# lachlants/denet

Hardware: AMD Instinct MI355X
Metric: images/sec train step, DeNet-34 skip 512x512 (higher is better)
Workload: dtype f32

## Files before the change

### denet_amd/csrc/winograd.hip

```cpp
#include "wino.h"
#include "bn_pointwise.h"
#include "../../include/denet_hip.h"

namespace {

template <int MO>
__global__ __launch_bounds__(256) void wino_input_kernel(const float* __restrict__ x, float* __restrict__ V, int N, int H,
                                                         int W, int C, int TH, int TW, long T, int up) {
    using WT = Wino<MO>;
    constexpr int TS = WT::TS;
    const int c4n = C / 4;
    const long idx = (long)blockIdx.x * 256 + threadIdx.x;
    if (idx >= T * c4n) return;
    const int c4 = (int)(idx % c4n);
    const long t = idx / c4n;
    const int tx = (int)(t % TW);
    const int ty = (int)((t / TW) % TH);
    const int n = (int)(t / ((long)TW * TH));
    const f32x4 z = {0.f, 0.f, 0.f, 0.f};
    f32x4 tt[TS][TS];
#pragma unroll
    for (int j = 0; j < TS; ++j) {
        const int ix = MO * tx - 1 + j;
        f32x4 d[TS];
#pragma unroll
        for (int i = 0; i < TS; ++i) {
            const int iy = MO * ty - 1 + i;
            const bool ok = ((unsigned)iy < (unsigned)H) && ((unsigned)ix < (unsigned)W);
            d[i] = ok ? ld4(x + (((long)n * (H >> up) + (iy >> up)) * (W >> up) + (ix >> up)) * C + c4 * 4) : z;
        }
        wino_input_col<MO>(d, tt, j);
    }
    wino_input_store<MO>(tt, V, T, t, C, c4 * 4);
}

struct BnFoldDev {
    const float* x;
    const float* aux;
    const float* y;
    const float* gamma;
    const float* beta;
    const float* mean;
    const float* invstd;
    const float* coef;
    float* out;
    int relu;
};

template <int MO, bool BWD>
struct PrepLds {
    static constexpr int BT = 4;
    static constexpr int CQ = 8;
    static constexpr int PB = BT * MO;
    static constexpr int PP = PB + 2;
    static constexpr int NT = BT * BT * CQ;
    static constexpr int PS = CQ + 1;
    static constexpr size_t LDS = (size_t)PP * PP * PS * sizeof(f32x4);
};

template <int MO, bool BWD>
__global__ __launch_bounds__(128) void wino_prep_lds_kernel(BnFoldDev f, float* __restrict__ V, float* __restrict__ dM, int N,
                                                            int H, int W, int C, int TH, int TW, long T, int BH, int BW) {
    using WT = Wino<MO>;
    using PL = PrepLds<MO, BWD>;
    static_assert(PL::NT == 128, "launch bounds");
    constexpr int TS = WT::TS, BT = PL::BT, CQ = PL::CQ, PB = PL::PB, PP = PL::PP, NT = PL::NT, PS = PL::PS;
    extern __shared__ __attribute__((aligned(16))) unsigned char prep_smem[];
    f32x4* patch = (f32x4*)prep_smem;
    const int tid = threadIdx.x;
    const int cq = tid % CQ;
    const int cblk = blockIdx.y;
    const int c = (cblk * CQ + cq) * 4;
    int b = blockIdx.x;
    const int bx = b % BW; b /= BW;
    const int by = b % BH;
    const int n = b / BH;
    const f32x4 z = {0.f, 0.f, 0.f, 0.f};
    BnQuad bq;
    bn_quad_load<false, true>(bq, f.gamma, f.beta, f.mean, f.invstd, c);
    if (BWD) bn_quad_load_coef(bq, f.coef, C, c);
    const int y0 = by * PB - 1, x0 = bx * PB - 1;
    constexpr int SLOTS = NT / CQ;
    constexpr int ROUNDS = (PP * PP + SLOTS - 1) / SLOTS;
    constexpr int UB = 7;
    for (int r0 = 0; r0 < ROUNDS; r0 += UB) {
        f32x4 xv[UB], av[UB], yv[UB];
        long off[UB];
        int pix[UB];
        bool ok[UB], inner[UB];
#pragma unroll
        for (int u = 0; u < UB; ++u) {
            const int p = (r0 + u) * SLOTS + tid / CQ;
            const int py = p / PP, px = p - py * PP;
            const int iy = y0 + py, ix = x0 + px;
            pix[u] = p;
            ok[u] = p < PP * PP && ((unsigned)iy < (unsigned)H) && ((unsigned)ix < (unsigned)W);
            inner[u] = py >= 1 && py <= PB && px >= 1 && px <= PB;
            off[u] = ok[u] ? (((long)n * H + iy) * W + ix) * C + c : (long)c;
            xv[u] = ld4(f.x + off[u]);
            if (BWD || f.aux) av[u] = ld4(f.aux + off[u]);
            if (BWD && f.relu && f.y) yv[u] = ld4(f.y + off[u]);
        }
#pragma unroll
        for (int u = 0; u < UB; ++u) {
            f32x4 d;
            if (!BWD) {
                d = bn_forward(bq, xv[u], f.aux != nullptr, av[u], f.relu);
                if (ok[u] && inner[u]) *(f32x4*)(f.out + off[u]) = d;
            } else {
                f32x4 g = av[u];
                if (f.relu) g = f.y ? bn_mask_y(g, yv[u]) : bn_mask_x(bq, g, xv[u]);
                d = bn_backward(bq, g, xv[u]);
                if (ok[u] && inner[u] && f.out) *(f32x4*)(f.out + off[u]) = g;
            }
            if (pix[u] < PP * PP) patch[pix[u] * PS + cq] = ok[u] ? d : z;
        }
    }
    __syncthreads();
    const int tl = tid / CQ;
    const int tyl = tl / BT, txl = tl - tyl * BT;
    const int ty = by * BT + tyl, tx = bx * BT + txl;
    if (ty >= TH || tx >= TW) return;
    const long t = ((long)n * TH + ty) * TW + tx;
    {
        f32x4 tt[TS][TS];
#pragma unroll
        for (int j = 0; j < TS; ++j) {
            f32x4 d[TS];
#pragma unroll
            for (int i = 0; i < TS; ++i) d[i] = patch[((MO * tyl + i) * PP + MO * txl + j) * PS + cq];
            wino_input_col<MO>(d, tt, j);
        }
        wino_input_store<MO>(tt, V, T, t, C, c);
    }
    if (BWD) {
        f32x4 a[TS][MO];
#pragma unroll
        for (int j = 0; j < MO; ++j) {
            f32x4 d[MO];
#pragma unroll
            for (int i = 0; i < MO; ++i) d[i] = patch[((MO * tyl + 1 + i) * PP + MO * txl + 1 + j) * PS + cq];
            wino_dout_col<MO>(d, a, j);
        }
        wino_dout_store<MO>(a, dM, T, t, C, c);
    }
}

template <int MO, bool BWD>
int launch_prep_lds(const BnFoldDev& f, float* V, float* dM, int N, int H, int W, int C, int TH, int TW, long T, hipStream_t stream) {
    using PL = PrepLds<MO, BWD>;
    static bool attr_set[DENET_MAX_DEVICES] = {};
    const hipError_t e = denet_allow_dynamic_lds((const void*)wino_prep_lds_kernel<MO, BWD>, (int)PL::LDS, attr_set);
    if (e != hipSuccess) {
        denet_set_error("conv_wino fold: hipFuncSetAttribute(%zu B LDS): %s", PL::LDS, hipGetErrorString(e));
        return -(int)e;
    }
    const int BH = (TH + PL::BT - 1) / PL::BT, BW = (TW + PL::BT - 1) / PL::BT;
    hipLaunchKernelGGL((wino_prep_lds_kernel<MO, BWD>), dim3((unsigned)(N * BH * BW), (unsigned)(C / (4 * PL::CQ))), dim3(PL::NT),
                       PL::LDS, stream, f, V, dM, N, H, W, C, TH, TW, T, BH, BW);
    return DENET_OK;
}

template <int MO>
__global__ __launch_bounds__(256) void wino_filter_kernel(const float* __restrict__ w, float* __restrict__ U, int K, int C) {
    using WT = Wino<MO>;
    constexpr int TS = WT::TS;
    const long idx = (long)blockIdx.x * 256 + threadIdx.x;
    if (idx >= (long)K * C) return;
    const int c = (int)(idx % C);
    const int k = (int)(idx / C);
    float g[3][3];
#pragma unroll
    for (int r = 0; r < 3; ++r)
#pragma unroll
        for (int s = 0; s < 3; ++s) g[r][s] = w[(((long)k * 3 + r) * 3 + s) * C + c];
    float u[TS][TS];
    wino_filter_transform<MO>(g, u);
    const long KC = (long)K * C;
#pragma unroll
    for (int i = 0; i < TS; ++i)
#pragma unroll
        for (int j = 0; j < TS; ++j) U[(long)(TS * i + j) * KC + (long)k * C + c] = u[i][j];
}

template <int MO>
__global__ __launch_bounds__(256) void wino_filter_dgrad_kernel(const float* __restrict__ w, float* __restrict__ U, int K,
                                                                int C) {
    using WT = Wino<MO>;
    constexpr int TS = WT::TS;
    __shared__ float tile[TS * TS][16][17];
    const int kl = threadIdx.x >> 4, cl = threadIdx.x & 15;
    const int k0 = blockIdx.y * 16, c0 = blockIdx.x * 16;
    {
        const int k = k0 + kl, c = c0 + cl;
        float g[3][3];
#pragma unroll
        for (int r = 0; r < 3; ++r)
#pragma unroll
            for (int q = 0; q < 3; ++q) g[r][q] = w[(((long)k * 3 + (2 - r)) * 3 + (2 - q)) * C + c];
        float u[TS][TS];
        wino_filter_transform<MO>(g, u);
#pragma unroll
        for (int i = 0; i < TS; ++i)
#pragma unroll
            for (int j = 0; j < TS; ++j) tile[TS * i + j][cl][kl] = u[i][j];
    }
    __syncthreads();
    const long KC = (long)K * C;
    const int co = threadIdx.x >> 4, ko = threadIdx.x & 15;
#pragma unroll
    for (int xi = 0; xi < TS * TS; ++xi) U[(long)xi * KC + (long)(c0 + co) * K + k0 + ko] = tile[xi][co][ko];
}

template <int MO>
__global__ __launch_bounds__(256) void wino_output_kernel(const float* __restrict__ Mx, const float* __restrict__ bias,
                                                          const float* __restrict__ add, float* __restrict__ y, int N,
                                                          int H, int W, int K, int TH, int TW, long T, int relu,
                                                          double* __restrict__ stats, BnFoldDev bs) {
    using WT = Wino<MO>;
    constexpr int TS = WT::TS;
    __shared__ double red[2][256][4];
    const int k4n = K / 4;
    const long idx = (long)blockIdx.x * 256 + threadIdx.x;
    const bool valid = idx < T * k4n;
    const f32x4 z = {0.f, 0.f, 0.f, 0.f};
    double dsum[4] = {0.0, 0.0, 0.0, 0.0}, dsq[4] = {0.0, 0.0, 0.0, 0.0};
    if (valid) {
        const int k4 = (int)(idx % k4n);
        const long t = idx / k4n;
        const int tx = (int)(t % TW);
        const int ty = (int)((t / TW) % TH);
        const int n = (int)(t / ((long)TW * TH));
        f32x4 s[MO][TS];
#pragma unroll
        for (int j = 0; j < TS; ++j) {
            f32x4 m[TS];
#pragma unroll
            for (int i = 0; i < TS; ++i) m[i] = ld4(Mx + ((long)(TS * i + j) * T + t) * K + k4 * 4);
            wino_output_col<MO>(m, s, j);
        }
        f32x4 b = z;
        if (bias) b = ld4(bias + k4 * 4);
        BnQuad bq = {};
        if (bs.x) bn_quad_load<true, true>(bq, bs.gamma, bs.beta, bs.mean, bs.invstd, k4 * 4);
#pragma unroll
        for (int i = 0; i < MO; ++i) {
            f32x4 ssum = z, ssq = z;
#pragma unroll
            for (int j = 0; j < MO; ++j) {
                f32x4 acc = wino_output_at<MO>(s[i], j);
                if (MO * ty + i >= H || MO * tx + j >= W) continue;
                const long o = (((long)n * H + MO * ty + i) * W + MO * tx + j) * K + k4 * 4;
                acc += b;
                if (add) acc += ld4(add + o);
                if (relu) {
                    acc[0] = fmaxf(acc[0], 0.f);
                    acc[1] = fmaxf(acc[1], 0.f);
                    acc[2] = fmaxf(acc[2], 0.f);
                    acc[3] = fmaxf(acc[3], 0.f);
                }
                *(f32x4*)(y + o) = acc;
                if (bs.x) {
                    const f32x4 xv = ld4(bs.x + o);
                    f32x4 g = acc;
                    if (bs.relu) g = bs.y ? bn_mask_y(g, ld4(bs.y + o)) : bn_mask_x(bq, g, xv);
                    ssum += g;
                    ssq += g * bn_xhat(bq, xv);
                } else {
                    ssum += acc;
                    ssq += acc * acc;
                }
            }
            if (stats) {
#pragma unroll
                for (int c = 0; c < 4; ++c) {
                    dsum[c] += (double)ssum[c];
                    dsq[c] += (double)ssq[c];
                }
            }
        }
    }
    if (!stats) return;
#pragma unroll
    for (int c = 0; c < 4; ++c) {
        red[0][threadIdx.x][c] = dsum[c];
        red[1][threadIdx.x][c] = dsq[c];
    }
    __syncthreads();
    for (int st = 128; st >= k4n; st >>= 1) {
        if ((int)threadIdx.x < st) {
#pragma unroll
            for (int c = 0; c < 4; ++c) {
                red[0][threadIdx.x][c] += red[0][threadIdx.x + st][c];
                red[1][threadIdx.x][c] += red[1][threadIdx.x + st][c];
            }
        }
        __syncthreads();
    }
    if ((int)threadIdx.x < k4n) {
        double* ps = stats + (long)blockIdx.x * 2 * K + threadIdx.x * 4;
#pragma unroll
        for (int c = 0; c < 4; ++c) {
            ps[c] = red[0][threadIdx.x][c];
            ps[K + c] = red[1][threadIdx.x][c];
        }
    }
}

template <int MO>
__global__ __launch_bounds__(256) void wino_dout_kernel(const float* __restrict__ dy, float* __restrict__ dM, int N, int H,
                                                        int W, int K, int TH, int TW, long T) {
    using WT = Wino<MO>;
    constexpr int TS = WT::TS;
    const int k4n = K / 4;
    const long idx = (long)blockIdx.x * 256 + threadIdx.x;
    if (idx >= T * k4n) return;
    const int k4 = (int)(idx % k4n);
    const long t = idx / k4n;
    const int tx = (int)(t % TW);
    const int ty = (int)((t / TW) % TH);
    const int n = (int)(t / ((long)TW * TH));
    const f32x4 z = {0.f, 0.f, 0.f, 0.f};
    f32x4 a[TS][MO];
#pragma unroll
    for (int j = 0; j < MO; ++j) {
        f32x4 d[MO];
#pragma unroll
        for (int i = 0; i < MO; ++i) {
            const int oy = MO * ty + i, ox = MO * tx + j;
            const bool in = oy < H && ox < W;
            const f32x4 v = ld4(dy + (((long)n * H + (in ? oy : 0)) * W + (in ? ox : 0)) * K + k4 * 4);
            d[i] = in ? v : z;
        }
        wino_dout_col<MO>(d, a, j);
    }
    wino_dout_store<MO>(a, dM, T, t, K, k4 * 4);
}

template <int MO>
__global__ __launch_bounds__(256) void wino_dfilter_kernel(const float* __restrict__ dU, float* __restrict__ dw, int K, int C) {
    using WT = Wino<MO>;
    constexpr int TS = WT::TS;
    const long idx = (long)blockIdx.x * 256 + threadIdx.x;
    if (idx >= (long)K * C) return;
    const int c = (int)(idx % C);
    const int k = (int)(idx / C);
    const long KC = (long)K * C;
    float r[3][TS];
#pragma unroll
    for (int j = 0; j < TS; ++j) {
        float u[TS];
#pragma unroll
        for (int i = 0; i < TS; ++i) u[i] = dU[(long)(TS * i + j) * KC + (long)k * C + c];
        wino_dfilter_col<MO>(u, r, j);
    }
    float g[3][3];
    wino_dfilter_rows<MO>(r, g);
#pragma unroll
    for (int i = 0; i < 3; ++i)
#pragma unroll
        for (int j = 0; j < 3; ++j) dw[(((long)k * 3 + i) * 3 + j) * C + c] = g[i][j];
}

struct WinoDims {
    int TS, NX, TH, TW;
    long T;
    size_t nU, nV, nM;
};

int wino_dims(int mo, int N, int H, int W, int C, int K, WinoDims* d) {
    DENET_CHECK_ARG(mo == 2 || mo == 4, "conv_wino: output tile must be 2 or 4 (got %d)", mo);
    DENET_CHECK_ARG(H > 0 && W > 0 && C % 32 == 0 && K % 32 == 0, "conv_wino: the channel counts must be multiples of 32");
    d->TS = mo + 2;
    d->NX = d->TS * d->TS;
    d->TH = (H + mo - 1) / mo;
    d->TW = (W + mo - 1) / mo;
    d->T = (long)N * d->TH * d->TW;
    d->nU = (size_t)d->NX * C * K;
    d->nV = (size_t)d->NX * d->T * C;
    d->nM = (size_t)d->NX * d->T * K;
    DENET_CHECK_ARG(d->T < (1L << 31) / d->NX, "conv_wino: too many tiles");
    return DENET_OK;
}

#define WINO_LAUNCH(MO_, KERNEL, NTHREADS, ...)                                                                       \
    {                                                                                                               \
        const unsigned blocks_ = (unsigned)(((NTHREADS) + 255) / 256);                                              \
        if ((MO_) == 2) hipLaunchKernelGGL(KERNEL<2>, dim3(blocks_), dim3(256), 0, stream, __VA_ARGS__);             \
        else hipLaunchKernelGGL(KERNEL<4>, dim3(blocks_), dim3(256), 0, stream, __VA_ARGS__);                        \
    }

int wino_filter(int mo, bool dgrad, const float* w, float* U, int K, int C, hipStream_t stream) {
    if (dgrad) {
        if (mo == 2) hipLaunchKernelGGL(wino_filter_dgrad_kernel<2>, dim3(C / 16, K / 16), dim3(256), 0, stream, w, U, K, C);
        else hipLaunchKernelGGL(wino_filter_dgrad_kernel<4>, dim3(C / 16, K / 16), dim3(256), 0, stream, w, U, K, C);
    } else {
        WINO_LAUNCH(mo, wino_filter_kernel, (long)K * C, w, U, K, C);
    }
    DENET_CHECK_LAUNCH("conv_wino filter transform");
    return DENET_OK;
}

int wino_run(int mo, bool dgrad, const float* in, const float* w, const float* u_cached, float* v_keep, const float* bias,
             const float* add, float* out, float* ws, size_t ws_bytes, int N, int H, int W, int Cin, int Cout,
             hipStream_t stream, int relu = 0, double* stats = nullptr, const BnFoldDev* fold = nullptr, float* dm_out = nullptr,
             hipEvent_t transform_done = nullptr, const BnFoldDev* out_sums = nullptr, int in_up = 0) {
    DENET_CHECK_ARG((in || fold) && w && out && ws, "conv_wino: null pointer");
    WinoDims d;
    int rc = wino_dims(mo, N, H, W, Cin, Cout, &d);
    if (rc) return rc;
    DENET_CHECK_ARG(ws_bytes >= (d.nU + d.nV + d.nM) * sizeof(float), "conv_wino: workspace too small (%zu < %zu)",
                    ws_bytes, (d.nU + d.nV + d.nM) * sizeof(float));
    float* Uw = ws;
    float* V = v_keep ? v_keep : Uw + d.nU;
    float* Mx = Uw + d.nU + d.nV;
    const long kc = (long)Cin * Cout;
    const float* U = u_cached;
    if (!U) {
        rc = dgrad ? wino_filter(mo, true, w, Uw, Cin, Cout, stream) : wino_filter(mo, false, w, Uw, Cout, Cin, stream);
        if (rc) return rc;
        U = Uw;
    }
    if (fold) {
        DENET_CHECK_ARG(!dgrad || dm_out, "conv_wino: the backward fold needs the dM buffer");
        if (dgrad) rc = mo == 2 ? launch_prep_lds<2, true>(*fold, V, dm_out, N, H, W, Cin, d.TH, d.TW, d.T, stream)
                                : launch_prep_lds<4, true>(*fold, V, dm_out, N, H, W, Cin, d.TH, d.TW, d.T, stream);
        else rc = mo == 2 ? launch_prep_lds<2, false>(*fold, V, nullptr, N, H, W, Cin, d.TH, d.TW, d.T, stream)
                          : launch_prep_lds<4, false>(*fold, V, nullptr, N, H, W, Cin, d.TH, d.TW, d.T, stream);
        if (rc) return rc;
    } else {
        WINO_LAUNCH(mo, wino_input_kernel, d.T * (Cin / 4), in, V, N, H, W, Cin, d.TH, d.TW, d.T, in_up);
    }
    DENET_CHECK_LAUNCH("conv_wino transforms");
    if (transform_done) {
        const hipError_t e = hipEventRecord(transform_done, stream);
        if (e != hipSuccess) {
            denet_set_error("conv_wino: hipEventRecord: %s", hipGetErrorString(e));
            return -(int)e;
        }
    }
    BnFoldDev bs = {};
    if (out_sums && stats) bs = *out_sums;
    if (const int tb4 = (H % mo == 0 && W % mo == 0) ? denet_wino4f_block(mo, d.T, Cin, Cout) : 0)
        return denet_wino4f_run(tb4, V, U, bias, add, out, stats, bs.x, bs.y, bs.gamma, bs.beta, bs.mean, bs.invstd, bs.relu, N, H, W,
                                Cin, Cout, relu, stream);
    rc = denet_gemm_batched_nt(V, U, Mx, d.NX, (int)d.T, Cout, Cin, d.T * Cin, kc, d.T * Cout, stream);
    if (rc) return rc;
    WINO_LAUNCH(mo, wino_output_kernel, d.T * (Cout / 4), Mx, bias, add, out, N, H, W, Cout, d.TH, d.TW, d.T, relu, stats, bs);
    DENET_CHECK_LAUNCH("conv_wino output");
    return DENET_OK;
}

int wino_stats_rows(int tile, int N, int H, int W, int Cin, int Kout, size_t stats_bytes) {
    const long T = (long)N * ((H + tile - 1) / tile) * ((W + tile - 1) / tile);
    long rows;
    if (const int tb4 = (H % tile == 0 && W % tile == 0) ? denet_wino4f_block(tile, T, Cin, Kout) : 0) rows = denet_wino4f_stats_rows(tb4, T);
    else {
        const int k4n = Kout / 4;
        if (!(k4n > 0 && k4n <= 256 && 256 % k4n == 0)) return 0;
        rows = (T * k4n + 255) / 256;
    }
    return stats_bytes >= (size_t)rows * 2 * Kout * sizeof(double) ? (int)rows : 0;
}

}

static int wino_wgrad_run(const float* x, const float* dy, const float* dm_ready, const float* v_cached, float* dw,
                          float* workspace, size_t workspace_bytes, float* split_ws, size_t split_ws_bytes, int tile, int N,
                          int H, int W, int C, int K, hipStream_t stream) {
    DENET_CHECK_ARG((x || v_cached) && (dy || dm_ready) && dw && workspace, "conv_wino_wgrad: null pointer");
    WinoDims d;
    int rc = wino_dims(tile, N, H, W, C, K, &d);
    if (rc) return rc;
    DENET_CHECK_ARG(workspace_bytes >= (d.nU + d.nV + d.nM) * sizeof(float), "conv_wino_wgrad: workspace too small");
    float* dU = workspace;
    const float* V = v_cached;
    float* dM = dU + d.nU + d.nV;
    if (!V) {
        float* Vw = dU + d.nU;
        WINO_LAUNCH(tile, wino_input_kernel, d.T * (C / 4), x, Vw, N, H, W, C, d.TH, d.TW, d.T, 0);
        V = Vw;
    }
    const float* dMr = dm_ready;
    if (!dMr) {
        WINO_LAUNCH(tile, wino_dout_kernel, d.T * (K / 4), dy, dM, N, H, W, K, d.TH, d.TW, d.T);
        dMr = dM;
    }
    DENET_CHECK_LAUNCH("conv_wino_wgrad transforms");
    const int sp = denet_wino4g_splits(tile, d.T, C, K);
    if (sp && (sp == 1 || (split_ws && split_ws_bytes >= denet_wino4g_workspace_bytes(sp, C, K))))
        rc = denet_wino4g_run(sp, dMr, V, dU, split_ws, split_ws_bytes, d.T, C, K, stream);
    else
        rc = denet_wgrad_batched(V, dMr, dU, split_ws, split_ws_bytes, d.NX, (int)d.T, C, K, stream);
    if (rc) return rc;
    WINO_LAUNCH(tile, wino_dfilter_kernel, (long)K * C, dU, dw, K, C);
    DENET_CHECK_LAUNCH("conv_wino_wgrad filter");
    return DENET_OK;
}

extern "C" int denet_conv_wino_wgrad(const float* x, const float* dy, const float* v_cached, float* dw, float* workspace,
                                     size_t workspace_bytes, float* split_ws, size_t split_ws_bytes, int tile, int N, int H,
                                     int W, int C, int K, hipStream_t stream) {
    DENET_CHECK_ARG(x && dy, "conv_wino_wgrad: null pointer");
    return wino_wgrad_run(x, dy, nullptr, v_cached, dw, workspace, workspace_bytes, split_ws, split_ws_bytes, tile, N, H, W, C, K,
                          stream);
}

extern "C" int denet_conv_wino_wgrad_dm(const float* x, const float* dm, const float* v_cached, float* dw, float* workspace,
                                        size_t workspace_bytes, float* split_ws, size_t split_ws_bytes, int tile, int N, int H,
                                        int W, int C, int K, hipStream_t stream) {
    DENET_CHECK_ARG(dm, "conv_wino_wgrad_dm: null pointer");
    return wino_wgrad_run(x, nullptr, dm, v_cached, dw, workspace, workspace_bytes, split_ws, split_ws_bytes, tile, N, H, W, C, K,
                          stream);
}

static int fold_from(const denet_bn_link* bn, bool bwd, BnFoldDev* f) {
    DENET_CHECK_ARG(bn && bn->x && bn->gamma && bn->mean && bn->invstd, "conv_wino fold: null pointer");
    DENET_CHECK_ARG(bwd ? (bn->aux && bn->coef && (!bn->relu || bn->y || bn->beta)) : (bn->beta && bn->out),
                    "conv_wino fold: incomplete batch-norm description");
    f->x = bn->x; f->aux = bn->aux; f->y = bn->y; f->gamma = bn->gamma; f->beta = bn->beta; f->mean = bn->mean;
    f->invstd = bn->invstd; f->coef = bn->coef; f->out = bn->out; f->relu = bn->relu;
    return DENET_OK;
}

extern "C" int denet_conv_wino_fwd_fold(const denet_bn_link* bn, const float* w, const float* u_cached, float* v_keep,
                                        const float* bias, const float* add, float* y, int relu, double* stats_partial,
                                        size_t stats_bytes, int* stats_rows, float* workspace, size_t workspace_bytes, int tile,
                                        int N, int H, int W, int C, int K, hipStream_t stream) {
    BnFoldDev f;
    int rc = fold_from(bn, false, &f);
    if (rc) return rc;
    double* st = nullptr;
    if (stats_partial) {
        DENET_CHECK_ARG(stats_rows && !relu, "conv_wino_fwd_fold: bad statistics arguments");
        *stats_rows = wino_stats_rows(tile, N, H, W, C, K, stats_bytes);
        st = *stats_rows ? stats_partial : nullptr;
    }
    return wino_run(tile, false, nullptr, w, u_cached, v_keep, bias, add, y, workspace, workspace_bytes, N, H, W, C, K, stream,
                    relu ? 1 : 0, st, &f);
}

static int sums_request(const denet_bn_link* sums_of, double* stats_partial, size_t stats_bytes, int* stats_rows, int tile, int N,
                        int H, int W, int C, int K, BnFoldDev* bs, double** st) {
    *st = nullptr;
    if (!sums_of) return DENET_OK;
    DENET_CHECK_ARG(stats_partial && stats_rows, "conv_wino dgrad: the backward sums need a buffer");
    DENET_CHECK_ARG(sums_of->x && sums_of->mean && sums_of->invstd && (!sums_of->relu || sums_of->y || (sums_of->gamma && sums_of->beta)),
                    "conv_wino dgrad: incomplete batch-norm description for the backward sums");
    *stats_rows = wino_stats_rows(tile, N, H, W, K, C, stats_bytes);
    if (*stats_rows) {
        *bs = BnFoldDev{};
        bs->x = sums_of->x; bs->y = sums_of->relu ? sums_of->y : nullptr; bs->gamma = sums_of->gamma; bs->beta = sums_of->beta;
        bs->mean = sums_of->mean; bs->invstd = sums_of->invstd; bs->relu = sums_of->relu;
        *st = stats_partial;
    }
    return DENET_OK;
}

extern "C" int denet_conv_wino_dgrad_fold(const denet_bn_link* bn, float* dm_out, const float* w, const float* u_cached,
                                          const float* add, float* dx, const denet_bn_link* sums_of, double* stats_partial,
                                          size_t stats_bytes, int* stats_rows, float* workspace, size_t workspace_bytes, int tile,
                                          int N, int H, int W, int C, int K, void* transform_done_event, hipStream_t stream) {
    BnFoldDev f, bs;
    double* st;
    int rc = fold_from(bn, true, &f);
    if (rc) return rc;
    rc = sums_request(sums_of, stats_partial, stats_bytes, stats_rows, tile, N, H, W, C, K, &bs, &st);
    if (rc) return rc;
    return wino_run(tile, true, nullptr, w, u_cached, nullptr, nullptr, add, dx, workspace, workspace_bytes, N, H, W, K, C, stream,
                    0, st, &f, dm_out, (hipEvent_t)transform_done_event, st ? &bs : nullptr);
}

extern "C" int denet_conv_wino_dgrad_sums(const float* dy, const float* w, const float* u_cached, const float* add, float* dx,
                                          const denet_bn_link* sums_of, double* stats_partial, size_t stats_bytes, int* stats_rows,
                                          float* workspace, size_t workspace_bytes, int tile, int N, int H, int W, int C, int K,
                                          hipStream_t stream) {
    BnFoldDev bs;
    double* st;
    int rc = sums_request(sums_of, stats_partial, stats_bytes, stats_rows, tile, N, H, W, C, K, &bs, &st);
    if (rc) return rc;
    return wino_run(tile, true, dy, w, u_cached, nullptr, nullptr, add, dx, workspace, workspace_bytes, N, H, W, K, C, stream, 0, st,
                    nullptr, nullptr, nullptr, st ? &bs : nullptr);
}

extern "C" int denet_conv_wino_tune(float* workspace, size_t workspace_bytes, float* split_ws, size_t split_ws_bytes,
                                    int tile, int N, int H, int W, int C, int K, hipStream_t stream) {
    DENET_CHECK_ARG(workspace, "conv_wino_tune: null workspace");
    WinoDims d;
    int rc = wino_dims(tile, N, H, W, C, K, &d);
    if (rc) return rc;
    DENET_CHECK_ARG(workspace_bytes >= (d.nU + d.nV + d.nM) * sizeof(float), "conv_wino_tune: workspace too small");
    float* U = workspace;
    (void)hipMemsetAsync(U, 0, (d.nU + d.nV + d.nM) * sizeof(float), stream);
    const long T = d.T;
    rc = denet_gemm_batched_tune(U + d.nU, U, U + d.nU + d.nV, d.NX, (int)T, K, C, T * C, (long)C * K, T * K, stream);
    if (rc) return rc;
    rc = denet_gemm_batched_tune(U + d.nU + d.nV, U, U + d.nU, d.NX, (int)T, C, K, T * K, (long)C * K, T * C, stream);
    if (rc || !split_ws) return rc;
    return denet_wgrad_batched_tune(U + d.nU, U + d.nU + d.nV, U, split_ws, split_ws_bytes, d.NX, (int)T, C, K, stream);
}

extern "C" size_t denet_conv_wino_workspace_bytes(int tile, int N, int H, int W, int C, int K) {
    const size_t nx = (size_t)(tile + 2) * (tile + 2);
    const size_t T = (size_t)N * ((H + tile - 1) / tile) * ((W + tile - 1) / tile);
    return (nx * C * K + nx * T * C + nx * T * K) * sizeof(float);
}

extern "C" int denet_conv_wino_fwd(const float* x, const float* w, const float* u_cached, float* v_keep, const float* bias,
                                   const float* add, float* y, float* workspace, size_t workspace_bytes, int tile, int N,
                                   int H, int W, int C, int K, hipStream_t stream) {
    return wino_run(tile, false, x, w, u_cached, v_keep, bias, add, y, workspace, workspace_bytes, N, H, W, C, K, stream);
}

extern "C" int denet_conv_wino_fwd_act(const float* x, const float* w, const float* u_cached, float* v_keep,
                                       const float* bias, const float* add, float* y, int relu, float* workspace,
                                       size_t workspace_bytes, int tile, int N, int H, int W, int C, int K,
                                       hipStream_t stream) {
    return wino_run(tile, false, x, w, u_cached, v_keep, bias, add, y, workspace, workspace_bytes, N, H, W, C, K, stream,
                    relu ? 1 : 0);
}

extern "C" int denet_conv_wino_fwd_stats_up(const float* x_small, const float* w, const float* u_cached, float* v_keep,
                                            const float* bias, const float* add, float* y, double* stats_partial,
                                            size_t stats_bytes, int* stats_rows, float* workspace, size_t workspace_bytes,
                                            int tile, int N, int H, int W, int C, int K, hipStream_t stream) {
    DENET_CHECK_ARG((tile == 2 || tile == 4) && H % 2 == 0 && W % 2 == 0, "conv_wino_fwd_stats_up: bad arguments");
    double* st = nullptr;
    if (stats_partial) {
        DENET_CHECK_ARG(stats_rows, "conv_wino_fwd_stats_up: null pointer");
        *stats_rows = wino_stats_rows(tile, N, H, W, C, K, stats_bytes);
        st = *stats_rows ? stats_partial : nullptr;
    }
    return wino_run(tile, false, x_small, w, u_cached, v_keep, bias, add, y, workspace, workspace_bytes, N, H, W, C, K, stream, 0, st,
                    nullptr, nullptr, nullptr, nullptr, 1);
}

extern "C" int denet_conv_wino_fwd_stats(const float* x, const float* w, const float* u_cached, float* v_keep,
                                         const float* bias, const float* add, float* y, double* stats_partial,
                                         size_t stats_bytes, int* stats_rows, float* workspace, size_t workspace_bytes,
                                         int tile, int N, int H, int W, int C, int K, hipStream_t stream) {
    DENET_CHECK_ARG(stats_partial && stats_rows && (tile == 2 || tile == 4), "conv_wino_fwd_stats: bad arguments");
    *stats_rows = wino_stats_rows(tile, N, H, W, C, K, stats_bytes);
    return wino_run(tile, false, x, w, u_cached, v_keep, bias, add, y, workspace, workspace_bytes, N, H, W, C, K, stream, 0,
                    *stats_rows ? stats_partial : nullptr);
}

extern "C" int denet_conv_wino_filter(const float* w, float* u, int tile, int dgrad, int C, int K, hipStream_t stream) {
    DENET_CHECK_ARG(w && u && (tile == 2 || tile == 4) && C > 0 && K > 0, "conv_wino_filter: bad arguments");
    DENET_CHECK_ARG(C % 16 == 0 && K % 16 == 0, "conv_wino_filter: the channel counts must be multiples of 16 (got C=%d K=%d)", C, K);
    return wino_filter(tile, dgrad != 0, w, u, K, C, stream);
}

extern "C" int denet_conv_wino_dgrad(const float* dy, const float* w, const float* u_cached, const float* add, float* dx,
                                     float* workspace, size_t workspace_bytes, int tile, int N, int H, int W, int C, int K,
                                     hipStream_t stream) {
    return wino_run(tile, true, dy, w, u_cached, nullptr, nullptr, add, dx, workspace, workspace_bytes, N, H, W, K, C, stream);
}
```

Before: 1091.

## Add wide 4x8-tile prep kernel variant for F(4,3) Winograd with swizzled LDS

Adds a WIDE variant of the BN-fold Winograd prep kernel that handles 4x8 tiles per block (256 threads) for the F(4x4,3x3) case when the tile width allows. The wider patch shares the one-pixel halo across more tiles, which cuts redundant global reads, and it raises the load unroll depth. The padded LDS stride is replaced by an XOR swizzle of adjacent pixel columns to avoid bank conflicts without padding. In exchange each block uses more LDS and threads, which may lower occupancy.

```diff
diff --git a/denet_amd/csrc/winograd.hip b/denet_amd/csrc/winograd.hip
--- a/denet_amd/csrc/winograd.hip
+++ b/denet_amd/csrc/winograd.hip
@@ -47,31 +47,36 @@
     int relu;
 };
 
-template <int MO, bool BWD>
+template <int MO, bool BWD, bool WIDE>
 struct PrepLds {
-    static constexpr int BT = 4;
+    static constexpr int BTY = 4, BTX = WIDE ? 8 : 4;
     static constexpr int CQ = 8;
-    static constexpr int PB = BT * MO;
-    static constexpr int PP = PB + 2;
-    static constexpr int NT = BT * BT * CQ;
-    static constexpr int PS = CQ + 1;
-    static constexpr size_t LDS = (size_t)PP * PP * PS * sizeof(f32x4);
+    static constexpr int PBY = BTY * MO, PBX = BTX * MO;
+    static constexpr int PPY = PBY + 2, PPX = PBX + 2;
+    static constexpr int NT = BTY * BTX * CQ;
+    static constexpr int PS = WIDE ? CQ : CQ + 1;
+    static constexpr int UB = WIDE ? 10 : 7;
+    static constexpr size_t LDS = (size_t)PPY * PPX * PS * sizeof(f32x4);
+    static __device__ __forceinline__ int at(int py, int px, int cq) {
+        return (py * PPX + (WIDE ? px ^ ((px >> 2) & 1) : px)) * PS + cq;
+    }
 };
 
-template <int MO, bool BWD>
-__global__ __launch_bounds__(128) void wino_prep_lds_kernel(BnFoldDev f, float* __restrict__ V, float* __restrict__ dM, int N,
-                                                            int H, int W, int C, int TH, int TW, long T, int BH, int BW) {
+template <int MO, bool BWD, bool WIDE>
+__global__ __launch_bounds__((PrepLds<MO, BWD, WIDE>::NT), (WIDE ? 2 : 1)) void wino_prep_lds_kernel(
+    BnFoldDev f, float* __restrict__ V, float* __restrict__ dM, int N, int H, int W, int C, int TH, int TW, long T, int BH, int BW) {
     using WT = Wino<MO>;
-    using PL = PrepLds<MO, BWD>;
-    static_assert(PL::NT == 128, "launch bounds");
-    constexpr int TS = WT::TS, BT = PL::BT, CQ = PL::CQ, PB = PL::PB, PP = PL::PP, NT = PL::NT, PS = PL::PS;
+    using PL = PrepLds<MO, BWD, WIDE>;
+    static_assert(PL::NT == 128 || PL::NT == 256, "launch bounds");
+    static_assert(PL::PPX % 2 == 0, "the pixel swap pairs columns inside a row");
+    constexpr int TS = WT::TS, BTX = PL::BTX, CQ = PL::CQ, PBY = PL::PBY, PBX = PL::PBX, PPY = PL::PPY, PPX = PL::PPX, NT = PL::NT;
     extern __shared__ __attribute__((aligned(16))) unsigned char prep_smem[];
     f32x4* patch = (f32x4*)prep_smem;
     const int tid = threadIdx.x;
     const int cq = tid % CQ;
     const int cblk = blockIdx.y;
+    int b = blockIdx.x;
     const int c = (cblk * CQ + cq) * 4;
-    int b = blockIdx.x;
     const int bx = b % BW; b /= BW;
     const int by = b % BH;
     const int n = b / BH;
@@ -79,23 +84,23 @@
     BnQuad bq;
     bn_quad_load<false, true>(bq, f.gamma, f.beta, f.mean, f.invstd, c);
     if (BWD) bn_quad_load_coef(bq, f.coef, C, c);
-    const int y0 = by * PB - 1, x0 = bx * PB - 1;
+    const int y0 = by * PBY - 1, x0 = bx * PBX - 1;
     constexpr int SLOTS = NT / CQ;
-    constexpr int ROUNDS = (PP * PP + SLOTS - 1) / SLOTS;
-    constexpr int UB = 7;
+    constexpr int ROUNDS = (PPY * PPX + SLOTS - 1) / SLOTS;
+    constexpr int UB = PL::UB;
     for (int r0 = 0; r0 < ROUNDS; r0 += UB) {
         f32x4 xv[UB], av[UB], yv[UB];
         long off[UB];
-        int pix[UB];
+        int pat[UB];
         bool ok[UB], inner[UB];
 #pragma unroll
         for (int u = 0; u < UB; ++u) {
             const int p = (r0 + u) * SLOTS + tid / CQ;
-            const int py = p / PP, px = p - py * PP;
+            const int py = p / PPX, px = p - py * PPX;
             const int iy = y0 + py, ix = x0 + px;
-            pix[u] = p;
-            ok[u] = p < PP * PP && ((unsigned)iy < (unsigned)H) && ((unsigned)ix < (unsigned)W);
-            inner[u] = py >= 1 && py <= PB && px >= 1 && px <= PB;
+            pat[u] = p < PPY * PPX ? PL::at(py, px, cq) : -1;
+            ok[u] = p < PPY * PPX && ((unsigned)iy < (unsigned)H) && ((unsigned)ix < (unsigned)W);
+            inner[u] = py >= 1 && py <= PBY && px >= 1 && px <= PBX;
             off[u] = ok[u] ? (((long)n * H + iy) * W + ix) * C + c : (long)c;
             xv[u] = ld4(f.x + off[u]);
             if (BWD || f.aux) av[u] = ld4(f.aux + off[u]);
@@ -113,13 +118,13 @@
                 d = bn_backward(bq, g, xv[u]);
                 if (ok[u] && inner[u] && f.out) *(f32x4*)(f.out + off[u]) = g;
             }
-            if (pix[u] < PP * PP) patch[pix[u] * PS + cq] = ok[u] ? d : z;
+            if (pat[u] >= 0) patch[pat[u]] = ok[u] ? d : z;
         }
     }
     __syncthreads();
     const int tl = tid / CQ;
-    const int tyl = tl / BT, txl = tl - tyl * BT;
-    const int ty = by * BT + tyl, tx = bx * BT + txl;
+    const int tyl = tl / BTX, txl = tl - tyl * BTX;
+    const int ty = by * PL::BTY + tyl, tx = bx * BTX + txl;
     if (ty >= TH || tx >= TW) return;
     const long t = ((long)n * TH + ty) * TW + tx;
     {
@@ -128,7 +133,7 @@
         for (int j = 0; j < TS; ++j) {
             f32x4 d[TS];
 #pragma unroll
-            for (int i = 0; i < TS; ++i) d[i] = patch[((MO * tyl + i) * PP + MO * txl + j) * PS + cq];
+            for (int i = 0; i < TS; ++i) d[i] = patch[PL::at(MO * tyl + i, MO * txl + j, cq)];
             wino_input_col<MO>(d, tt, j);
         }
         wino_input_store<MO>(tt, V, T, t, C, c);
@@ -139,26 +144,34 @@
         for (int j = 0; j < MO; ++j) {
             f32x4 d[MO];
 #pragma unroll
-            for (int i = 0; i < MO; ++i) d[i] = patch[((MO * tyl + 1 + i) * PP + MO * txl + 1 + j) * PS + cq];
+            for (int i = 0; i < MO; ++i) d[i] = patch[PL::at(MO * tyl + 1 + i, MO * txl + 1 + j, cq)];
             wino_dout_col<MO>(d, a, j);
         }
         wino_dout_store<MO>(a, dM, T, t, C, c);
     }
 }
 
-template <int MO, bool BWD>
-int launch_prep_lds(const BnFoldDev& f, float* V, float* dM, int N, int H, int W, int C, int TH, int TW, long T, hipStream_t stream) {
-    using PL = PrepLds<MO, BWD>;
+template <int MO, bool BWD, bool WIDE>
+int launch_prep_lds_shape(const BnFoldDev& f, float* V, float* dM, int N, int H, int W, int C, int TH, int TW, long T, hipStream_t stream) {
+    using PL = PrepLds<MO, BWD, WIDE>;
     static bool attr_set[DENET_MAX_DEVICES] = {};
-    const hipError_t e = denet_allow_dynamic_lds((const void*)wino_prep_lds_kernel<MO, BWD>, (int)PL::LDS, attr_set);
+    const hipError_t e = denet_allow_dynamic_lds((const void*)wino_prep_lds_kernel<MO, BWD, WIDE>, (int)PL::LDS, attr_set);
     if (e != hipSuccess) {
         denet_set_error("conv_wino fold: hipFuncSetAttribute(%zu B LDS): %s", PL::LDS, hipGetErrorString(e));
         return -(int)e;
     }
-    const int BH = (TH + PL::BT - 1) / PL::BT, BW = (TW + PL::BT - 1) / PL::BT;
-    hipLaunchKernelGGL((wino_prep_lds_kernel<MO, BWD>), dim3((unsigned)(N * BH * BW), (unsigned)(C / (4 * PL::CQ))), dim3(PL::NT),
-                       PL::LDS, stream, f, V, dM, N, H, W, C, TH, TW, T, BH, BW);
+    const int BH = (TH + PL::BTY - 1) / PL::BTY, BW = (TW + PL::BTX - 1) / PL::BTX;
+    const dim3 grid((unsigned)(N * BH * BW), (unsigned)(C / (4 * PL::CQ)));
+    hipLaunchKernelGGL((wino_prep_lds_kernel<MO, BWD, WIDE>), grid, dim3(PL::NT), PL::LDS, stream, f, V, dM, N, H, W, C, TH, TW, T,
+                       BH, BW);
     return DENET_OK;
+}
+
+template <int MO, bool BWD>
+int launch_prep_lds(const BnFoldDev& f, float* V, float* dM, int N, int H, int W, int C, int TH, int TW, long T, hipStream_t stream) {
+    if constexpr (MO == 4)
+        if (TW >= PrepLds<MO, BWD, true>::BTX) return launch_prep_lds_shape<MO, BWD, true>(f, V, dM, N, H, W, C, TH, TW, T, stream);
+    return launch_prep_lds_shape<MO, BWD, false>(f, V, dM, N, H, W, C, TH, TW, T, stream);
 }
 
 template <int MO>
```

Result: no change. 1099, median of 6 (+0.7%).
